# rhinempi/Reflexiv

Hardware: AMD Instinct MI355X
Metric: k-mers/sec (extract+count+filter; wall-clock to final contigs beside it) (higher is better)
Workload: dtype u64; 1 GPU; synthetic 5 Gbp in all (5 Gbp per GPU x 1), E.coli-like genome 4640000 bp (1078x), PE150, k=31, -cover 30, 0.5% substitutions; reads_per_gpu=33333334, kmer_instances_per_gpu=4000000080, distinct_kmers=352952250, kmers_kept=4639950, parallelism=1 GPU

## Files before the change

### reflexiv_amd/api.py

```python
from __future__ import annotations

import ctypes as C
from dataclasses import dataclass

import time

import numpy as np

from . import _lib
from ._lib import Params, CRecords, RfxError, TWIN_DS, TWIN_RDD, RFX_OK, RFX_E_CAP


def _p(a):
    return a.ctypes.data_as(C.c_void_p) if a is not None else None


def _cap_error(where, need, detail) -> RfxError:
    e = RfxError(RFX_E_CAP, where, detail)
    e.need = int(need)
    return e


@dataclass
class Records:
# ... 1426 lines not shown
    def comm_destroy(self):
        if getattr(self, "comm", None):
            self.L.rfx_comm_destroy(self.comm)
            self.comm = None

    def comm_all_reduce(self, vals, op: str = "sum"):
        a = (C.c_int64 * len(vals))(*[int(v) for v in vals])
        self._check(self.L.rfx_comm_all_reduce_i64(self.comm, a, len(vals), 0 if op == "sum" else 1), "rfx_comm_all_reduce_i64")
        return [int(x) for x in a]

    def sharded_count_dev(self, d_words: int, n_reads: int, words_per_read: int, read_len: int, k: int, d_out_keys: int,
                          d_out_counts: int, cap: int, min_cov=2, max_cov=10_000_000, twin=TWIN_DS, generations=4,
                          front_clip=0, end_clip=0, d_read_len: int = 0):
        n = C.c_int64(0)
        tot = (C.c_int64 * 3)()
        st = self.L.rfx_dev_sharded_count(self.ctx, self.comm, C.c_void_p(d_words), C.c_void_p(d_read_len), C.c_int64(n_reads), words_per_read,
                                          read_len, k, front_clip, end_clip, generations, min_cov, max_cov, twin,
                                          C.c_void_p(d_out_keys), C.c_void_p(d_out_counts), C.c_int64(cap), C.byref(n), tot)
        if st == RFX_E_CAP:
            e = RfxError(st, "rfx_dev_sharded_count", f"needs room for {n.value} survivors, cap is {cap}")
            e.need = int(n.value)
            raise e
        self._check(st, "rfx_dev_sharded_count")
        return int(n.value), [int(x) for x in tot]

    def sharded_assemble_dev(self, d_keys: int, d_counts: int, n: int, prm: Params, gather_below: int = -1, text_cap: int = None):
        trace = np.zeros(prm.max_iter + 8, np.int64)
        cap = (1 << 20) + 64 * max(n, 1) if text_cap is None else int(text_cap)
        self.text_retries = 0
        while True:
            buf = np.empty(max(cap, 1), np.uint8)
            ln, nc, ntr = C.c_int64(0), C.c_int64(0), C.c_int64(0)
            st = self.L.rfx_dev_sharded_assemble(self.ctx, self.comm, C.c_void_p(d_keys), C.c_void_p(d_counts), C.c_int64(n), C.byref(prm),
                                                 C.c_int64(gather_below), _p(buf), C.c_int64(cap), C.byref(ln), C.byref(nc), _p(trace),
                                                 C.c_int64(len(trace)), C.byref(ntr))
            if st == RFX_E_CAP and ln.value > cap:
                cap = int(ln.value)
                self.text_retries += 1
                continue
            self._check(st, "rfx_dev_sharded_assemble")
            return bytes(buf[:ln.value]).decode(), int(nc.value), [int(x) for x in trace[:ntr.value]]

    def sharded_assemble_reads(self, bases, read_off, prm: Params, generations: int = 4, text_cap: int = None, gather_below: int = -1):
        bases = np.ascontiguousarray(bases, np.uint8)
        read_off = np.ascontiguousarray(read_off, np.int64)
        n_reads = len(read_off) - 1
        trace = np.zeros(prm.max_iter + 8, np.int64)
        tot = (C.c_int64 * 3)()
        cap = 3 * len(bases) + (1 << 20) if text_cap is None else int(text_cap)
        self.text_retries = 0
        while True:
            buf = np.empty(max(cap, 1), np.uint8)
            ln, nc, ntr = C.c_int64(0), C.c_int64(0), C.c_int64(0)
            st = self.L.rfx_sharded_assemble_reads(self.ctx, self.comm, _p(bases), _p(read_off), C.c_int64(n_reads), C.byref(prm),
                                                   generations, C.c_int64(gather_below), _p(buf), C.c_int64(cap), C.byref(ln), C.byref(nc), _p(trace),
                                                   C.c_int64(len(trace)), C.byref(ntr), tot)
            if st == RFX_E_CAP and ln.value > cap:
                cap = int(ln.value)
                self.text_retries += 1
                continue
            self._check(st, "rfx_sharded_assemble_reads")
            return (bytes(buf[:ln.value]).decode(), int(nc.value), [int(x) for x in trace[:ntr.value]], [int(x) for x in tot])

    def comm_bytes_bucketed(self) -> int:
        return int(self.L.rfx_comm_last_bytes_bucketed(self.comm))

    def gather_shards_dev(self, d_keys: int, d_counts: int, n: int, key_words: int, count_bytes: int, root: int,
                          d_out_keys: int, d_out_counts: int, cap: int) -> int:
        m = C.c_int64(0)
        st = self.L.rfx_dev_gather_shards(self.ctx, self.comm, C.c_void_p(d_keys), C.c_void_p(d_counts), C.c_int64(n), key_words,
                                          count_bytes, root, C.c_void_p(d_out_keys), C.c_void_p(d_out_counts), C.c_int64(cap),
                                          C.byref(m))
        if st == RFX_E_CAP:
            e = RfxError(st, "rfx_dev_gather_shards", f"needs room for {m.value} entries, cap is {cap}")
            e.need = int(m.value)
            raise e
        self._check(st, "rfx_dev_gather_shards")
        return int(m.value)

    def count_timing(self):
        out = {}
        for name in ("hist1", "part1", "hist2", "part2", "hist3", "part3", "leaf", "sort", "extract_w", "count_w",
                     "pair_hist", "pair_part", "stat_leaves", "stat_passes", "stat_overflows", "stat_l2_spilled", "stat_l2_void", "stat_l2_sweeps",
                     "stat_records"):
            ms, ln = C.c_float(0), C.c_int64(0)
            if self.L.rfx_last_count_timing(self.ctx, name.encode(), C.byref(ms), C.byref(ln)) == RFX_OK:
                out[name] = (float(ms.value), int(ln.value))
        return out
```

### reflexiv_amd/csrc/rfx_kmer.hip

```cpp
#include "rfx_internal.h"
#include "rfx_device.h"
#include <algorithm>
#include <cmath>
#include <cstdlib>

using namespace rfxd;

namespace {


__device__ __forceinline__ uint64_t nuc_code(uint8_t c) {
    return c == 'A' ? 0 : c == 'C' ? 1 : c == 'G' ? 2 : 3;
}

__global__ void k_encode(const uint8_t *__restrict__ bases, const int64_t *__restrict__ read_off,
                         int64_t n_reads, int wpr, uint64_t *__restrict__ words,
                         uint32_t *__restrict__ read_len) {
    int64_t t = (int64_t)blockIdx.x * blockDim.x + threadIdx.x;
    if (t >= n_reads * wpr) return;
    int64_t r = t / wpr;
    int w = (int)(t % wpr);
    int64_t b0 = read_off[r];
    int64_t len = read_off[r + 1] - b0;
    if (w == 0 && read_len) read_len[r] = (uint32_t)len;
// ... 356 lines not shown
constexpr int LT = 768;
constexpr int LEAF_WAVES_PER_EU = 6;
constexpr int RSLOTS = 768;
constexpr int RPROBE = 4;
constexpr int LOBUF = 512;
constexpr int LOBUF1 = 128;
constexpr int WSTAGE = 160;
constexpr int LSTAGE = WSTAGE * (LT / 64);
constexpr int LCAP_BITS = 12;
constexpr int LCAP = 1 << LCAP_BITS;
__device__ __forceinline__ uint32_t leaf_slot(uint32_t g) { return g >> (32 - LCAP_BITS); }
__device__ __forceinline__ uint32_t leaf_step(uint32_t g) { return ((g >> 8) & (LCAP - 1)) | 1u; }
__device__ __forceinline__ uint32_t leaf_next(uint32_t slot, uint32_t step) { return (slot + step) & (LCAP - 1); }
constexpr int LPROBE = 48;
constexpr uint64_t EMPTY = ~0ULL;
constexpr int LSTACK = 48;
constexpr int LB = 8;
constexpr int PBLOCK = 8192;
constexpr unsigned long long NOBLK = ~0ULL;

struct CountOut {
    unsigned long long n_out;
    unsigned long long n_distinct;
    unsigned long long n_failed;
    unsigned long long n_passes;
    unsigned long long n_overflow;
    unsigned long long n_leaves;
};

struct alignas(16) Rec { uint64_t w0, w1; };
__device__ __forceinline__ int rec_len(const Rec &r) { return (int)((r.w1 >> 32) & 15) + 1; }
struct alignas(32) WRec { uint64_t b0, b1, b2, hd; };
__device__ __forceinline__ int rec_len(const WRec &r) { return (int)((r.hd >> 32) & 15) + 1; }
__device__ __forceinline__ uint32_t rec_hdr(const Rec &r) { return (uint32_t)r.w1; }

template <int ELEM> struct LeafElem;
template <> struct LeafElem<0> {
    using T = uint64_t;
    static constexpr int PER_LANE = LB;
    __device__ static __forceinline__ T none() { return 0; }
    __device__ static __forceinline__ uint64_t key(const T &e) { return e; }
    __device__ static __forceinline__ uint32_t weight(const T &) { return 1u; }
    template <class F> __device__ static __forceinline__ void for_each_kmer(const T &e, int, F &&f) { f(e); }
};
template <> struct LeafElem<2> {
    using T = Rec;
    static constexpr int PER_LANE = LB / 2;
    __device__ static __forceinline__ T none() { return Rec{0, 0}; }
    __device__ static __forceinline__ uint64_t key(const T &e) { return e.w0; }
    __device__ static __forceinline__ uint32_t weight(const T &e) { return (uint32_t)e.w1; }
};
template <> struct LeafElem<1> {
    using T = Rec;
    static constexpr int PER_LANE = 1;
    __device__ static __forceinline__ T none() { return Rec{0, 0}; }
    __device__ static __forceinline__ uint64_t key(const T &e) { return e.w0; }
    __device__ static __forceinline__ uint32_t weight(const T &) { return 1u; }
    template <class F> __device__ static __forceinline__ void for_each_kmer(const T &e, int k, F &&f) {
        const int n = rec_len(e);
        const int k2 = 2 * k;
        uint64_t fwd = e.w0 >> (64 - k2);
        uint64_t rc = revcomp(fwd, k);
        uint64_t rest = (e.w0 << k2) | (e.w1 >> (64 - k2));
        const uint64_t mask = low_mask(k);
        const int top = k2 - 2;
        for (int i = 0; i < n; i++) {
            f(fwd < rc ? fwd : rc);
            const uint64_t b = rest >> 62;
            rest <<= 2;
            fwd = ((fwd << 2) | b) & mask;
            rc = (rc >> 2) | ((b ^ 3) << top);
        }
    }
};

__device__ __forceinline__ uint32_t wave_incl_scan(uint32_t x) {
    x += (uint32_t)__builtin_amdgcn_update_dpp(0, (int)x, 0x111, 0xf, 0xf, false);
    x += (uint32_t)__builtin_amdgcn_update_dpp(0, (int)x, 0x112, 0xf, 0xf, false);
    x += (uint32_t)__builtin_amdgcn_update_dpp(0, (int)x, 0x114, 0xf, 0xf, false);
    x += (uint32_t)__builtin_amdgcn_update_dpp(0, (int)x, 0x118, 0xf, 0xf, false);
    x += (uint32_t)__builtin_amdgcn_update_dpp(0, (int)x, 0x142, 0xa, 0xf, false);
    x += (uint32_t)__builtin_amdgcn_update_dpp(0, (int)x, 0x143, 0xc, 0xf, false);
    return x;
}

template <int ELEM, int KC = 0>
__global__ __launch_bounds__(LT, LEAF_WAVES_PER_EU) void k_leaf_count(const typename LeafElem<ELEM>::T *__restrict__ keys,
                                                   const uint64_t *__restrict__ leaf_off, const uint64_t *__restrict__ leaf_end, int64_t nleaf,
                                                   const uint64_t *__restrict__ sl_begin, const uint64_t *__restrict__ sl_end,
                                                   uint64_t heavy, uint64_t n_elems, int k_rt,
                                                   int min_cov, int max_cov, int apply_filter,
                                                   uint64_t *__restrict__ out_keys, int32_t *__restrict__ out_counts,
                                                   unsigned long long cap, CountOut *__restrict__ co,
                                                   int pair_out, uint32_t presplit) {
    constexpr bool RECS = ELEM == 1;
    const int k = KC ? KC : k_rt;
    __shared__ __attribute__((aligned(16))) unsigned long long tkey[LCAP];
    __shared__ __attribute__((aligned(16))) uint32_t tcnt[LCAP];
    constexpr int OB1 = RECS ? LOBUF1 : LOBUF;
    constexpr int OB2 = RECS ? (LSTAGE * 8) / 12 : 0;
    constexpr int OBT = OB1 + OB2;
    __shared__ unsigned long long obk[OB1];
    __shared__ int32_t obc[OB1];
    __shared__ uint32_t stackS[LSTACK], stacks[LSTACK];
    __shared__ int sp;
    __shared__ uint32_t overflow, ob_n, ob_lim;
    __shared__ unsigned long long g_emit;
    __shared__ unsigned long long blk_base, blk_next;
    __shared__ uint32_t blk_pos, have_next, need_grab;
    __shared__ uint32_t ps_eff;
    __shared__ __attribute__((aligned(16))) uint64_t stage[RECS ? LSTAGE : 2];
    unsigned long long *const obk2 = (unsigned long long *)stage;
    int32_t *const obc2 = (int32_t *)(obk2 + OB2);
    auto ob_put = [&](uint32_t i, unsigned long long key, int32_t c) __attribute__((always_inline)) {
        if (OB2 == 0 || i < (uint32_t)OB1) { obk[i] = key; obc[i] = c; }
        else { obk2[i - OB1] = key; obc2[i - OB1] = c; }
    };
    static_assert(RSLOTS == 64 * (LT / 64), "one block of record slots per wave");
    __shared__ unsigned long long rA[RECS ? RSLOTS : 1], rBC[RECS ? RSLOTS : 1];
    __shared__ uint32_t agg_on, agg_saved, agg_total;
    uint32_t my_distinct = 0;
    unsigned long long my_passes = 0, my_overflows = 0;
    const int lane_ = threadIdx.x & 63;
    const int wave_ = threadIdx.x >> 6;
    constexpr int NW = LT / 64;

    const int64_t l0 = (int64_t)(((unsigned long long)blockIdx.x * (unsigned long long)nleaf) / gridDim.x);
    const int64_t l1 = (int64_t)(((unsigned long long)(blockIdx.x + 1) * (unsigned long long)nleaf) / gridDim.x);
    if (l0 >= l1) return;
    const uint64_t stream_end = n_elems;
    auto range = [&](int64_t l, uint64_t &b, uint64_t &e) __attribute__((always_inline)) {
        if (sl_begin) { b = sl_begin[l]; e = sl_end[l]; return; }
        b = leaf_off[l]; e = leaf_end[l];
        if (heavy && e - b > heavy) e = b;
    };

    for (int i = threadIdx.x; i < LCAP; i += LT) { tkey[i] = EMPTY; tcnt[i] = 0; }
    if constexpr (RECS) for (int i = threadIdx.x; i < RSLOTS; i += LT) { rA[i] = EMPTY; rBC[i] = EMPTY; }
    if (threadIdx.x == 0) {
        ob_n = 0; ob_lim = 0xffffffffu; overflow = 0; sp = 0;
        blk_base = NOBLK; blk_next = NOBLK; blk_pos = PBLOCK; have_next = 0; need_grab = 1;
        ps_eff = presplit ? presplit : 0xffffffffu;
        agg_on = 1; agg_saved = 0; agg_total = 0;
    }

    auto flush = [&]() {
        __syncthreads();
        const uint32_t cntv = ob_n < ob_lim ? ob_n : ob_lim;
        if (ob_n == 0) return;
        if (threadIdx.x == 0 && cntv) g_emit = atomicAdd(&co->n_out, (unsigned long long)cntv);
        __syncthreads();
        for (uint32_t i = threadIdx.x; i < cntv; i += LT) {
            const unsigned long long pos = g_emit + i;
            if (pos < cap) {
                const bool own = OB2 == 0 || i < (uint32_t)OB1;
                const unsigned long long key = own ? obk[i] : obk2[i - OB1];
                const int32_t c = own ? obc[i] : obc2[i - OB1];
                if (pair_out) ((Rec *)out_keys)[pos] = Rec{key, (uint64_t)(uint32_t)c};
                else { out_keys[pos] = key; out_counts[pos] = c; }
            }
        }
        __syncthreads();
        if (threadIdx.x == 0) { ob_n = 0; ob_lim = 0xffffffffu; }
        __syncthreads();
    };

// ... 1113 lines not shown
constexpr int OS_CSTRIDE = 16;
constexpr int OS_MAXG = 512;
constexpr int OS_HOLES = 3;
struct OneSweep {
    const uint64_t *reg_start;
    const uint32_t *reg_cap;
    unsigned long long *cursor;
    uint64_t *holes;
    int *overflow;
    uint64_t total;
    unsigned long long *tile_counter;
    uint32_t ose, ose_shift;
};

template <int W, int SEG = 16, bool WIDE = false>
__global__ __launch_bounds__(SKT) void k_sk_sample_hist(ReadSrc s, Level lv, int sample, unsigned long long *__restrict__ hist) {
    __shared__ uint32_t h[1 << MAX_BITS];
    const int nb = 1 << lv.bits;
    for (int i = threadIdx.x; i < nb; i += SKT) h[i] = 0;
    __syncthreads();
    const int64_t ntile = (s.n_threads + SKT - 1) / SKT;
    for (int64_t T = (int64_t)blockIdx.x * sample; T < ntile; T += (int64_t)gridDim.x * sample) {
        const int64_t g = T * SKT + threadIdx.x;
        const bool in = g < s.n_threads;
        SegPos q{0, 0};
        int nk_r = 0;
        uint64_t w[3] = {0, 0, 0}, hi, lo;
        if (in) {
            q.r = g / s.segs;
            q.sgm = (int)(g - q.r * s.segs);
            seg_load<SEG>(s, q, w);
            nk_r = read_nk<WIDE>(s, q.r);
        }
        if (SEG == 32 || in)
            seg_runs<W, SEG == 32, SEG>(s, nk_r, q.sgm, w, [&](int, int, uint32_t canon) { atomicAdd(&h[sk_digit(canon, lv)], 1u); }, &hi, &lo);
    }
    __syncthreads();
    for (int i = threadIdx.x; i < nb; i += SKT) if (h[i]) atomicAdd(&hist[i], (unsigned long long)h[i]);
}

__global__ __launch_bounds__(1024) void k_plan_regions(const unsigned long long *__restrict__ hist, int nb, double scale, int G, int cap_pct,
                                                       double tiles,
                                                       uint64_t *__restrict__ reg_start, uint32_t *__restrict__ reg_cap,
                                                       unsigned long long *__restrict__ cursor, unsigned long long *__restrict__ totals) {
    __shared__ uint64_t caps[1 << MAX_BITS];
    __shared__ unsigned long long busiest;
    __shared__ uint32_t ose_s;
    const int d = threadIdx.x;
    if (d == 0) busiest = 0;
    __syncthreads();
    if (d < nb) atomicMax(&busiest, hist[d]);
    __syncthreads();
    if (d == 0) {
        const double per_tile = (double)busiest * scale / tiles;
        ose_s = per_tile <= 16.0 ? 64u : per_tile <= 32.0 ? 128u : per_tile <= 64.0 ? 256u : 0u;
    }
    __syncthreads();
    const uint32_t E = ose_s ? ose_s : OSE_MIN;
    if (d < nb) {
        const double c = (double)hist[d];
        const double est = c * scale;
        double room = (est + 6.0 * scale * sqrt(c + 1.0) + est / 64.0 + 1024.0) * (double)cap_pct / 100.0;
        uint64_t cap = (uint64_t)room + (uint64_t)G * OS_HOLES * E;
        cap = (cap + E - 1) / E * E;
        if (cap > 0xFFFFFF00ULL) cap = 0xFFFFFF00ULL / E * E;
        caps[d] = cap;
        reg_cap[d] = (uint32_t)cap;
    }
    __syncthreads();
    if (threadIdx.x == 0) {
        uint64_t at = 0;
        for (int i = 0; i < nb; i++) { reg_start[i] = at; cursor[(size_t)i * OS_CSTRIDE] = at; at += caps[i]; }
        reg_start[nb] = at;
        totals[0] = at + E;
        totals[1] = 0;
        totals[2] = ose_s;
    }
}

template <int SEG, bool WIDE> struct OsGeo {
    static constexpr int T = SEG > 16 && !WIDE ? 512 : SKT;
};
template <int W, bool WIDE = false, int SEG = 16>
__global__ __launch_bounds__((OsGeo<SEG, WIDE>::T), WIDE || SEG > 16 ? 4 : 8) void k_sk_onesweep(ReadSrc s, Level lv, OneSweep os,
                                                               std::conditional_t<WIDE, WRec, Rec> *__restrict__ out) {
    using RT = std::conditional_t<WIDE, WRec, Rec>;
    constexpr int SKT = OsGeo<SEG, WIDE>::T;
    extern __shared__ __attribute__((aligned(32))) unsigned char sk_smem[];
    const int nb = 1 << lv.bits;
#define buf ((RT *)sk_smem)
#define tail ((uint32_t *)(sk_smem + (size_t)nb * SKB * sizeof(RT)))
#define head (tail + nb)
#define cstart (tail + 2 * nb)
#define cbase (tail + 3 * nb)
#define nbase (tail + 4 * nb)
#define pbase (tail + 5 * nb)
    constexpr uint32_t DUMP = 0xFFFFFFFFu;
    const uint32_t OSE = os.ose, OSH = os.ose_shift;
    const uint64_t dump_at = os.total - OSE;
    auto grab = [&](int d) __attribute__((always_inline)) -> uint32_t {
        const unsigned long long b = atomicAdd(&os.cursor[(size_t)d * OS_CSTRIDE], (unsigned long long)OSE);
        return b + OSE <= dump_at ? (uint32_t)(b >> OSH) : DUMP;
    };
    auto phys = [&](uint32_t v, uint32_t cs, uint32_t cb, uint32_t nx) __attribute__((always_inline)) -> uint64_t {
        const uint32_t o = v - cs;
        const uint32_t b = o < (uint32_t)OSE ? cb : nx;
        return (b == DUMP ? dump_at : (uint64_t)b << OSH) + (o & (OSE - 1));
    };
    constexpr uint32_t NONE = 0xFFFFFFFEu;
    for (int i = threadIdx.x; i < nb; i += SKT) {
        tail[i] = 0; head[i] = 0; cstart[i] = 0;
        cbase[i] = grab(i);
        nbase[i] = grab(i);
        pbase[i] = grab(i);
    }
    __syncthreads();
    constexpr int LPB = SEG > 16 || WIDE ? 4 : SKB;
    auto drain = [&](bool final) __attribute__((always_inline)) {
#pragma nounroll
        for (int d = threadIdx.x / LPB; d < nb; d += SKT / LPB) {
            const int j = threadIdx.x % LPB;
            const uint32_t h = head[d], t = tail[d], cs = cstart[d], cb = cbase[d], nx = nbase[d];
            uint32_t e, nh;
            if (t - h > (uint32_t)SKB) { e = h + SKB; nh = t; }
            else {
                e = final ? t : (t & ~(uint32_t)(SKA - 1));
                if (e < h) e = h;
                nh = e;
            }
#pragma unroll
            for (int q = 0; q < SKB / LPB; q++) {
                const uint32_t g = h + j + q * LPB;
                if (g < e) out[phys(g, cs, cb, nx)] = buf[(size_t)d * SKB + (g & (SKB - 1))];
            }
            if (j == 0) {
                head[d] = nh;
                if (nh - cs >= (uint32_t)OSE) {
                    uint32_t c = cs, b0 = cb, b1 = nx, b2 = pbase[d];
                    while (nh - c >= (uint32_t)OSE) { c += OSE; b0 = b1; b1 = b2 != NONE ? b2 : grab(d); b2 = NONE; }
                    cstart[d] = c; cbase[d] = b0; nbase[d] = b1; pbase[d] = b2;
                }
            }
        }
    };
    __shared__ long long tile_lds[2];
    const int64_t ntile = (s.n_threads + SKT - 1) / SKT;
    const int my_d = (int)threadIdx.x;
    int64_t T = blockIdx.x;
    for (int rnd = 0; T < ntile; rnd++) {
        long long t_next = 0;
        if (threadIdx.x == SKT - 1) t_next = (long long)gridDim.x + (long long)atomicAdd(os.tile_counter, 1ULL);
        const bool ask = my_d < nb && pbase[my_d] == NONE;
        uint32_t req = DUMP;
        if (ask) req = grab(my_d);
        const int64_t g = T * SKT + threadIdx.x;
        const bool in = g < s.n_threads;
        SegPos q{0, 0};
        int nk_r = 0;
        uint64_t w[3] = {0, 0, 0}, hi = 0, lo = 0;
        uint32_t past = 0;
        if (in) {
            q.r = g / s.segs;
            q.sgm = (int)(g - q.r * s.segs);
            seg_load<SEG>(s, q, w);
            nk_r = read_nk<WIDE>(s, q.r);
        }
        if (SEG == 32 || in) {
            seg_runs<W, true, SEG>(s, nk_r, q.sgm, w, [&](int i0, int n, uint32_t canon) {
                const uint64_t hh = mmer_hash64(canon);
                const uint32_t hdr = (uint32_t)((hh << OWNER_BITS) >> 32);
                const unsigned d = lv.n_owners > 0 ? (((unsigned)__umul64hi(hh, (uint64_t)lv.n_owners) << lv.sub_bits) | (hdr >> (32 - lv.sub_bits)))
                                                   : rec_digit(hdr, 0, lv.bits);
                RT r;
                if constexpr (WIDE) {
                    const uint64_t *gw = s.words + q.r * s.wpr;
                    const int p = s.fc - s.wfl + q.sgm * SEG + i0;
                    const int wi = p >> 5, sft = 2 * (p & 31), last = s.wpr - 1;
                    const uint64_t a0 = gw[wi < last ? wi : last], a1 = gw[wi + 1 < last ? wi + 1 : last];
                    const uint64_t a2 = gw[wi + 2 < last ? wi + 2 : last], a3 = gw[wi + 3 < last ? wi + 3 : last];
                    r.b0 = sft ? (a0 << sft) | (a1 >> (64 - sft)) : a0;
                    r.b1 = sft ? (a1 << sft) | (a2 >> (64 - sft)) : a1;
                    r.b2 = sft ? (a2 << sft) | (a3 >> (64 - sft)) : a2;
                    r.hd = ((uint64_t)(n - 1) << 32) | (uint64_t)hdr;
                } else {
                    const int sft = 2 * i0;
                    const uint64_t x = (uint64_t)past << 32;
                    r.w0 = sft ? (hi << sft) | (lo >> (64 - sft)) : hi;
                    r.w1 = ((sft ? (lo << sft) | (x >> (64 - sft)) : lo) & 0xFFFFFFF000000000ULL) | ((uint64_t)(n - 1) << 32) | (uint64_t)hdr;
                }
                const uint32_t pos = atomicAdd(&tail[d], 1u);
                if (pos - head[d] < (uint32_t)SKB) buf[(size_t)d * SKB + (pos & (SKB - 1))] = r;
                else {
                    const uint32_t cs = cstart[d];
                    if (pos - cs < 2u * OSE) out[phys(pos, cs, cbase[d], nbase[d])] = r;
                    else *os.overflow = 1;
                }
            }, &hi, &lo, nullptr, &past);
        }
        if (threadIdx.x == SKT - 1) tile_lds[rnd & 1] = t_next;
        if (ask) pbase[my_d] = req;
        __syncthreads();
        drain(false);
        T = tile_lds[rnd & 1];
        __syncthreads();
    }
    drain(true);
    __syncthreads();
    for (int d = threadIdx.x; d < nb; d += SKT) {
        const uint32_t used = tail[d] - cstart[d], cb = cbase[d], nx = nbase[d], px = pbase[d];
        uint64_t *hl = os.holes + ((size_t)d * gridDim.x + blockIdx.x) * OS_HOLES;
        hl[0] = cb != DUMP && used < OSE ? ((((uint64_t)cb << OSH) + used) << 16) | (uint64_t)(OSE - used) : 0;
        hl[1] = nx != DUMP ? (((uint64_t)nx << OSH) << 16) | (uint64_t)OSE : 0;
        hl[2] = px != DUMP && px != NONE ? (((uint64_t)px << OSH) << 16) | (uint64_t)OSE : 0;
    }
}
#undef buf
#undef tail
#undef head
#undef cstart
#undef cbase
#undef nbase
#undef pbase

constexpr int FH_T = 1024;
template <class RT>
__global__ __launch_bounds__(FH_T) void k_fix_holes(OneSweep os, int G, RT *__restrict__ out, uint64_t *__restrict__ seg_begin,
                                                   uint64_t *__restrict__ seg_end, unsigned long long *__restrict__ totals) {
    constexpr int NHMAX = 2048;
    static_assert(NHMAX >= OS_HOLES * OS_MAXG && NHMAX % FH_T == 0, "holes per bucket");
    constexpr int NWMAX = NHMAX * OSE_MAX / 32;
    __shared__ uint32_t hstart[NHMAX], hoff[NHMAX + 1];
    __shared__ uint32_t bitmap[NWMAX];
    __shared__ uint32_t wsum[FH_T / 64];
    const int d = blockIdx.x;
    const int NH = OS_HOLES * G;
    const uint64_t base = os.reg_start[d];
    const unsigned long long alloc = os.cursor[(size_t)d * OS_CSTRIDE] - base;
    if (alloc > (unsigned long long)os.reg_cap[d]) {
        if (threadIdx.x == 0) { seg_begin[d] = base; seg_end[d] = base; *os.overflow = 1; }
        return;
    }
    auto block_excl_scan = [&](uint32_t v, uint32_t *total) __attribute__((always_inline)) -> uint32_t {
        const int lane = threadIdx.x & 63, wave = threadIdx.x >> 6;
        uint32_t x = v;
#pragma unroll
        for (int o = 1; o < 64; o <<= 1) { const uint32_t y = __shfl_up(x, o, 64); if (lane >= o) x += y; }
        if (lane == 63) wsum[wave] = x;
        __syncthreads();
        uint32_t b = 0, tot = 0;
        for (int i = 0; i < FH_T / 64; i++) { const uint32_t sv = wsum[i]; if (i < wave) b += sv; tot += sv; }
        __syncthreads();
        *total = tot;
        return b + x - v;
    };
    constexpr int HPT = NHMAX / FH_T;
    uint32_t hs[HPT], hl[HPT];
    uint32_t mine = 0;
#pragma unroll
    for (int r = 0; r < HPT; r++) {
        const int t = threadIdx.x * HPT + r;
        const uint64_t x = t < NH ? os.holes[(size_t)d * NH + t] : 0;
        hl[r] = (uint32_t)(x & 0xFFFFu);
        hs[r] = hl[r] ? (uint32_t)((x >> 16) - base) : 0u;
        mine += hl[r];
    }
    uint32_t H;
    block_excl_scan(mine, &H);
    const uint32_t size = (uint32_t)alloc - H;
    const uint32_t nw = (H + 31) / 32;
    const uint32_t wpt = (nw + FH_T - 1) / FH_T;
    for (uint32_t i = threadIdx.x; i < nw; i += FH_T) bitmap[i] = 0;
    __syncthreads();
    uint32_t fill[HPT], fsum = 0;
#pragma unroll
    for (int r = 0; r < HPT; r++) {
        fill[r] = hs[r] < size ? (hs[r] + hl[r] <= size ? hl[r] : size - hs[r]) : 0u;
        fsum += fill[r];
        for (uint32_t p = hs[r] + fill[r]; p < hs[r] + hl[r]; p++) atomicOr(&bitmap[(p - size) >> 5], 1u << ((p - size) & 31));
    }
    uint32_t F;
    uint32_t fo = block_excl_scan(fsum, &F);
#pragma unroll
    for (int r = 0; r < HPT; r++) {
        const int t = threadIdx.x * HPT + r;
        hstart[t] = hs[r]; hoff[t] = fo; fo += fill[r];
    }
// ... 255 lines not shown
            else return level_digit<MODE>(Rec{a.x, a.y}, used, lv);
        };
#define RCL_COUNT(i) { const uint64_t idx = c0 + (uint64_t)(i) * WCT + threadIdx.x; d##i = digit_of(q##i, w##i); if (idx < qe) atomicAdd(&h[d##i], 1u); }
        RCL_COUNT(0) RCL_COUNT(1) RCL_COUNT(2) RCL_COUNT(3)
#undef RCL_COUNT
        __syncthreads();
        for (int d = threadIdx.x; d < nb; d += WCT) {
            const uint32_t c = h[d];
            const uint64_t rs = pl.reg_start[d], re = pl.reg_start[d + 1];
            unsigned long long base = 0;
            if (c) base = atomicAdd(&pl.cursor[d], (unsigned long long)c);
            tail[d] = head[d] = rs + base;
            lim[d] = re;
        }
        __syncthreads();
#define RCL_PUT(i) { const uint64_t idx = c0 + (uint64_t)(i) * WCT + threadIdx.x; \
            if (idx < qe) { \
                const unsigned d = d##i; \
                const unsigned long long g = atomicAdd(&tail[d], 1ULL); \
                if (g >= lim[d]) {  } \
                else if (g - head[d] < (unsigned long long)B) { V *to = (V *)buf + ((size_t)d * B + (g & (B - 1))) * NV; to[0] = q##i; if constexpr (NV == 2) to[1] = w##i; } \
                else { V *to = (V *)out + g * NV; to[0] = q##i; if constexpr (NV == 2) to[1] = w##i; } \
            } }
        RCL_PUT(0) RCL_PUT(1) RCL_PUT(2) RCL_PUT(3)
#undef RCL_PUT
        __syncthreads();
        drain(true);
        __syncthreads();
    }
}

constexpr int L2S_STRIDE = 16;
struct L2Plan {
    const uint64_t *seg_begin, *seg_end; const uint64_t *child_start; int *flags;
    void *spill_rec; uint32_t *spill_child; unsigned long long *spill_cursor; uint32_t spill_cap;
    unsigned long long *tail_cursor; uint64_t out_cap;
};
template <int MODE>
__global__ __launch_bounds__(PT) void k_l2_sample(const typename LevelElem<MODE>::T *__restrict__ recs, L2Plan pl, Level lv, int used,
                                                  uint32_t *__restrict__ sampled) {
    __shared__ uint32_t h[1 << MAX_BITS];
    const int p = blockIdx.x, nb = 1 << lv.bits;
    for (int i = threadIdx.x; i < nb; i += PT) h[i] = 0;
    __syncthreads();
    const uint64_t qb = pl.seg_begin[p], qe = pl.seg_end[p];
    for (uint64_t c = (uint64_t)blockIdx.y * L2S_STRIDE; c * PT < qe - qb; c += (uint64_t)gridDim.y * L2S_STRIDE) {
        const uint64_t i = qb + c * PT + threadIdx.x;
        if (i < qe) {
            const typename LevelElem<MODE>::T r = recs[i];
            if constexpr (MODE == 2) { if (r.w1 == 0) continue; }
            atomicAdd(&h[level_digit<MODE>(r, used, lv)], 1u);
        }
    }
    __syncthreads();
    for (int i = threadIdx.x; i < nb; i += PT) if (h[i]) atomicAdd(&sampled[(int64_t)p * nb + i], h[i]);
}
__global__ void k_l2_caps(const uint32_t *__restrict__ sampled, int64_t nchild, uint32_t *__restrict__ ccap, int pct) {
    const int64_t c = (int64_t)blockIdx.x * blockDim.x + threadIdx.x;
    if (c >= nchild) return;
    const float s = (float)sampled[c];
    uint32_t C = (uint32_t)((float)L2S_STRIDE * (s + 6.0f * sqrtf(s + 1.0f) + 32.0f));
    if (pct != 100) C = (uint32_t)((uint64_t)C * (uint64_t)pct / 100u);
    ccap[c] = (C + 7u) & ~7u;
}
__global__ __launch_bounds__(1024) void k_l2_check(L2Plan pl, int nseg, int64_t nchild, uint64_t out_cap) {
    __shared__ unsigned long long sum_n, mx_n;
    if (threadIdx.x == 0) { sum_n = 0; mx_n = 0; }
    __syncthreads();
    if ((int)threadIdx.x < nseg) {
        const unsigned long long n = pl.seg_end[threadIdx.x] - pl.seg_begin[threadIdx.x];
        atomicAdd(&sum_n, n);
        atomicMax(&mx_n, n);
    }
    __syncthreads();
    if (threadIdx.x == 0) {
        const unsigned long long mean = sum_n / (unsigned long long)(nseg > 0 ? nseg : 1);
        pl.flags[0] = (pl.child_start[nchild] + 8ULL * pl.spill_cap + 65536ULL > out_cap || mx_n > mean + mean / 2 + 4096) ? 1 : 0;
        pl.flags[1] = 0;
        *pl.spill_cursor = 0;
        *pl.tail_cursor = (pl.child_start[nchild] + 7ULL) & ~7ULL;
    }
}

typedef unsigned long long l2_v2 __attribute__((ext_vector_type(2)));
template <class RT>
__device__ __forceinline__ RT l2_load_stream(const RT *p) {
    static_assert(sizeof(RT) == 16 || sizeof(RT) == 32, "16- or 32-byte records");
    const l2_v2 a = __builtin_nontemporal_load((const l2_v2 *)p);
    if constexpr (sizeof(RT) == 32) {
        const l2_v2 b = __builtin_nontemporal_load((const l2_v2 *)p + 1);
        return RT{a.x, a.y, b.x, b.y};
    } else return RT{a.x, a.y};
}
template <class RT>
__device__ __forceinline__ void l2_store_stream(RT *p, const RT &r) {
    const uint64_t *w = (const uint64_t *)&r;
    __builtin_nontemporal_store(l2_v2{w[0], w[1]}, (l2_v2 *)p);
    if constexpr (sizeof(RT) == 32) __builtin_nontemporal_store(l2_v2{w[2], w[3]}, (l2_v2 *)p + 1);
}
template <int B, int MODE>
__global__ __launch_bounds__(WCT) void k_rec_l2sweep(const typename LevelElem<MODE>::T *__restrict__ recs, L2Plan pl, Level lv, int used,
                                                     typename LevelElem<MODE>::T *__restrict__ out, uint64_t *__restrict__ leaf_end) {
    using Rec = typename LevelElem<MODE>::T;
    extern __shared__ __attribute__((aligned(32))) unsigned char wc_smem[];
    constexpr int A = B / 2;
    if (pl.flags[0]) return;
    const int p = blockIdx.x;
    const int nb = 1 << lv.bits;
    const uint64_t qb = pl.seg_begin[p], qe = pl.seg_end[p];
    Rec *buf = (Rec *)wc_smem;
    unsigned long long *tail = (unsigned long long *)(buf + (size_t)nb * B);
    unsigned long long *head = tail + nb;
    unsigned long long *lim = head + nb;
    for (int i = threadIdx.x; i < nb; i += WCT) {
        tail[i] = head[i] = pl.child_start[(int64_t)p * nb + i];
        lim[i] = pl.child_start[(int64_t)p * nb + i + 1];
    }
    __syncthreads();
    auto drain = [&](bool final) __attribute__((always_inline)) {
#pragma nounroll
        for (int d = threadIdx.x / B; d < nb; d += WCT / B) {
            const int j = threadIdx.x % B;
            const unsigned long long h = head[d], lm = lim[d];
            unsigned long long t = tail[d];
            if (t > lm) t = lm;
            unsigned long long e, nh;
            if (t - h > (unsigned long long)B) { e = h + B; nh = t; }
            else {
                e = final ? t : (t & ~(unsigned long long)(A - 1));
                if (e < h) e = h;
                nh = e;
            }
            const unsigned long long g = h + j;
            if (g < e) l2_store_stream(out + g, buf[(size_t)d * B + (g & (B - 1))]);
            if (j == 0) head[d] = nh;
        }
    };
    for (uint64_t b0 = qb; b0 < qe; b0 += (uint64_t)WCT * WC_PER) {
        Rec r[WC_PER];
#pragma unroll
        for (int i = 0; i < WC_PER; i++) {
            const uint64_t idx = b0 + (uint64_t)i * WCT + threadIdx.x;
            r[i] = l2_load_stream(recs + (idx < qe ? idx : qe - 1));
        }
#pragma unroll
        for (int i = 0; i < WC_PER; i++) {
            const uint64_t idx = b0 + (uint64_t)i * WCT + threadIdx.x;
            bool live = idx < qe;
            if constexpr (MODE == 2) live = live && r[i].w1 != 0;
            if (live) {
                const unsigned d = level_digit<MODE>(r[i], used, lv);
                const unsigned long long g = atomicAdd(&tail[d], 1ULL);
                if (g >= lim[d]) {
                    const unsigned long long sk = atomicAdd(pl.spill_cursor, 1ULL);
                    if (sk < (unsigned long long)pl.spill_cap) { ((Rec *)pl.spill_rec)[sk] = r[i]; pl.spill_child[sk] = (uint32_t)(p * nb + (int)d); }
                    else pl.flags[1] = 1;
                }
                else if (g - head[d] < (unsigned long long)B) buf[(size_t)d * B + (g & (B - 1))] = r[i];
                else out[g] = r[i];
            }
        }
        __syncthreads();
        drain(false);
        __syncthreads();
    }
    drain(true);
    __syncthreads();
    for (int d = threadIdx.x; d < nb; d += WCT) leaf_end[(int64_t)p * nb + d] = tail[d];
}

constexpr int L2F_T = 1024, L2F_SLOTS = 2048, L2F_MAXC = 1536;
template <class RT>
__global__ __launch_bounds__(L2F_T) void k_l2_spill_fix(L2Plan pl, uint64_t *__restrict__ cstart, uint64_t *__restrict__ lend, RT *__restrict__ out) {
    __shared__ uint32_t tkey[L2F_SLOTS], tcnt[L2F_SLOTS], tfill[L2F_SLOTS], tcap[L2F_SLOTS];
    __shared__ unsigned long long tbase[L2F_SLOTS];
    __shared__ uint32_t ndistinct;
    __shared__ int bad;
    if (pl.flags[0] || pl.flags[1]) return;
    const unsigned long long ns = *pl.spill_cursor;
    if (ns == 0) return;
    constexpr uint32_t NOKEY = 0xFFFFFFFFu;
    for (int i = threadIdx.x; i < L2F_SLOTS; i += L2F_T) { tkey[i] = NOKEY; tcnt[i] = 0; tfill[i] = 0; }
// ... 743 lines not shown
    const int OST = seg32 ? OsGeo<32, false>::T : SKT;
    const int64_t ntile = ceil_div(rsrc.n_threads, OST);
    const int64_t ntile_s = ceil_div(rsrc.n_threads, SKT);
    const int per_cu = WIDE ? 1 : 2;
    const int G = (int)std::max<int64_t>(1, std::min<int64_t>(std::min<int64_t>(OS_MAXG, (int64_t)ctx->num_cu * per_cu),
                                                                std::max<int64_t>(std::min<int64_t>(ntile, 64), ntile / 32)));
    int sample = 32;
    if (ntile_s < 64 * (int64_t)sample) sample = (int)std::max<int64_t>(1, ntile_s / 64);
    const int64_t n_sampled = ceil_div(ntile_s, sample);
    const int cap_pct = getenv("RFX_SK_ONESWEEP_CAP") ? std::max(1, atoi(getenv("RFX_SK_ONESWEEP_CAP"))) : 100;
    DevBuf hist, reg_start, reg_cap, cursor, totals, holes;
    RFX_HIP(hist.alloc((size_t)nb * 8 + 16, ctx->stream));
    RFX_ALLOC(reg_start, uint64_t, nb + 1);
    RFX_ALLOC(reg_cap, uint32_t, nb);
    RFX_ALLOC(cursor, unsigned long long, (size_t)nb * OS_CSTRIDE);
    RFX_HIP(totals.alloc(24, ctx->stream));
    RFX_ALLOC(holes, uint64_t, (size_t)nb * OS_HOLES * G);
    RFX_HIP(hipMemsetAsync(hist.p, 0, (size_t)nb * 8 + 16, ctx->stream));
    int *d_overflow = (int *)(hist.as<unsigned long long>() + nb);
    {
        ScopedTimer t(ctx, hn);
        const dim3 gs((unsigned)std::min<int64_t>(n_sampled, (int64_t)ctx->num_cu * 8));
        if constexpr (WIDE) {
            if (W == 18) RFX_LAUNCH((k_sk_sample_hist<18, 16, true>), gs, dim3(SKT), 0, rsrc, lv, sample, hist.as<unsigned long long>());
            else RFX_LAUNCH((k_sk_sample_hist<19, 16, true>), gs, dim3(SKT), 0, rsrc, lv, sample, hist.as<unsigned long long>());
        } else switch (W) {
#define X(w) case w: if (seg32) RFX_LAUNCH((k_sk_sample_hist<w, 32>), gs, dim3(SKT), 0, rsrc, lv, sample, hist.as<unsigned long long>()); \
                     else RFX_LAUNCH((k_sk_sample_hist<w>), gs, dim3(SKT), 0, rsrc, lv, sample, hist.as<unsigned long long>()); break;
            RFX_SK_W_CASES(X)
            default: X(19)
#undef X
        }
        RFX_LAUNCH(k_plan_regions, dim3(1), dim3(1024), 0, hist.as<unsigned long long>(), nb,
                   (double)ntile_s / (double)n_sampled, G, cap_pct, (double)ntile, reg_start.as<uint64_t>(), reg_cap.as<uint32_t>(),
                   cursor.as<unsigned long long>(), totals.as<unsigned long long>());
    }
    unsigned long long h_tot[3] = {0, 0, 0};
    RFX_HIP(hipMemcpyAsync(h_tot, totals.p, 24, hipMemcpyDeviceToHost, ctx->stream));
    RFX_TRY(sync_checked(ctx));
    const uint32_t ose = (uint32_t)h_tot[2];
    if (ose == 0) {
        if (getenv("RFX_TRACE")) fprintf(stderr, "one-sweep level 1: not tried (the sample puts too much on one bucket)\n");
        return RFX_OK;
    }
    int ose_shift = 0;
    while ((1u << ose_shift) < ose) ose_shift++;
    Rec *dst = d_dst;
    if (d_dst) {
        if ((int64_t)h_tot[0] > cap_dst) { *n_recs = (int64_t)h_tot[0]; return RFX_E_CAP; }
    } else {
        dst = (Rec *)ctx->ws_get(ws_slot, (size_t)h_tot[0] * sizeof(Rec));
        if (!dst) { ctx->last_error = "workspace allocation failed"; return RFX_E_HIP; }
    }
    const OneSweep os{reg_start.as<uint64_t>(), reg_cap.as<uint32_t>(), cursor.as<unsigned long long>(), holes.as<uint64_t>(), d_overflow,
                      (uint64_t)h_tot[0], hist.as<unsigned long long>() + nb + 1, ose, (uint32_t)ose_shift};
    const size_t lds = (size_t)nb * (SKB * sizeof(Rec) + 24);
    {
        ScopedTimer t(ctx, pn);
        if constexpr (WIDE) {
            if (W == 18) {
                RFX_HIP(hipFuncSetAttribute((const void *)k_sk_onesweep<18, true>, hipFuncAttributeMaxDynamicSharedMemorySize, (int)lds));
                RFX_LAUNCH((k_sk_onesweep<18, true>), dim3((unsigned)G), dim3(SKT), lds, rsrc, lv, os, dst);
            } else {
                RFX_HIP(hipFuncSetAttribute((const void *)k_sk_onesweep<19, true>, hipFuncAttributeMaxDynamicSharedMemorySize, (int)lds));
                RFX_LAUNCH((k_sk_onesweep<19, true>), dim3((unsigned)G), dim3(SKT), lds, rsrc, lv, os, dst);
            }
        } else {
            switch (W) {
#define X(w) case w: if (seg32) { \
                         RFX_HIP(hipFuncSetAttribute((const void *)k_sk_onesweep<w, false, 32>, hipFuncAttributeMaxDynamicSharedMemorySize, (int)lds)); \
                         RFX_LAUNCH((k_sk_onesweep<w, false, 32>), dim3((unsigned)G), dim3(OST), lds, rsrc, lv, os, dst); \
                     } else { \
                         RFX_HIP(hipFuncSetAttribute((const void *)k_sk_onesweep<w>, hipFuncAttributeMaxDynamicSharedMemorySize, (int)lds)); \
                         RFX_LAUNCH((k_sk_onesweep<w>), dim3((unsigned)G), dim3(SKT), lds, rsrc, lv, os, dst); \
                     } break;
                RFX_SK_W_CASES(X)
                default: X(19)
#undef X
            }
        }
        RFX_LAUNCH(k_fix_holes<Rec>, dim3((unsigned)nb), dim3(FH_T), 0, os, G, dst, d_seg_begin, d_seg_end,
                   totals.as<unsigned long long>());
    }
    int h_over = 0;
    RFX_HIP(hipMemcpyAsync(h_tot, totals.p, 16, hipMemcpyDeviceToHost, ctx->stream));
    RFX_HIP(hipMemcpyAsync(&h_over, d_overflow, 4, hipMemcpyDeviceToHost, ctx->stream));
    RFX_TRY(sync_checked(ctx));
    if (getenv("RFX_TRACE"))
        fprintf(stderr, "one-sweep level 1: %llu records in regions of %llu (sample 1/%d, %d workgroups, extents of %u)%s\n", h_tot[1], h_tot[0], sample, G, ose,
                h_over ? " -- a region overflowed: two passes instead" : "");
    if (h_over == 2) { ctx->last_error = "one-sweep level 1: holes and tail records do not balance"; return RFX_E_STATE; }
    if (h_over) return RFX_OK;
    *out_recs = dst;
    *n_recs = (int64_t)h_tot[1];
    ctx->timing["stat_records"].launches += (int64_t)h_tot[1];
    *done = true;
    return RFX_OK;
}

template <int MODE>
static int records_resweep(rfx_ctx *ctx, const typename LevelElem<MODE>::T *recs, int64_t n_recs, const Level &lv, int used, int oslot,
                           uint64_t *d_seg_begin, uint64_t *d_seg_end, const typename LevelElem<MODE>::T **out_recs, bool *done,
                           const char *hn, const char *pn) {
    using RT = typename LevelElem<MODE>::T;
    *done = false;
    const int mode = getenv("RFX_REC_ONESWEEP") ? atoi(getenv("RFX_REC_ONESWEEP")) : (MODE == 0 || MODE == 3 ? 1 : 0);
    if (MODE == 2 || !mode || lv.bits < 4 || lv.bits > 9 || lv.n_owners > 0 || (mode != 2 && n_recs < ((int64_t)1 << 24))) return RFX_OK;
    const int nb = 1 << lv.bits;
    constexpr int B = MODE == 3 ? 8 : 16;
    if (nb > 256 && B * sizeof(RT) * nb + 28 * (size_t)nb > 160 * 1024) return RFX_OK;
    const size_t lds = (size_t)nb * (B * sizeof(RT) + 28);
    const int64_t nchunk = ceil_div(n_recs, PT);
    int sample = 32;
    if (nchunk < 256 * (int64_t)sample) sample = (int)std::max<int64_t>(1, nchunk / 256);
    const int64_t n_sampled = ceil_div(nchunk, sample);
    DevBuf hist, reg_start, cursor;
    RFX_HIP(hist.alloc((size_t)nb * 8 + 8, ctx->stream));
    RFX_ALLOC(reg_start, uint64_t, nb + 1);
    RFX_ALLOC(cursor, unsigned long long, nb);
    RFX_HIP(hipMemsetAsync(hist.p, 0, (size_t)nb * 8 + 8, ctx->stream));
    const ClaimPlan pl{reg_start.as<uint64_t>(), cursor.as<unsigned long long>(), (int *)(hist.as<unsigned long long>() + nb)};
    {
        ScopedTimer t(ctx, hn);
        RFX_LAUNCH(k_rec_sample_hist<MODE>, dim3((unsigned)std::min<int64_t>(n_sampled, (int64_t)ctx->num_cu * 8)), dim3(PT), 0,
                   recs, (uint64_t)n_recs, lv, used, sample, hist.as<unsigned long long>());
        RFX_LAUNCH(k_claim_plan, dim3(1), dim3(1024), 0, hist.as<unsigned long long>(), nb,
                   (double)nchunk / (double)n_sampled, pl);
    }
    uint64_t total = 0;
    RFX_HIP(hipMemcpyAsync(&total, reg_start.as<uint64_t>() + nb, 8, hipMemcpyDeviceToHost, ctx->stream));
    RFX_TRY(sync_checked(ctx));
    if ((int64_t)total > 2 * n_recs + ((int64_t)1 << 26)) return RFX_OK;
    RT *dst = (RT *)ctx->ws_get(oslot, (size_t)total * sizeof(RT));
    if (!dst) { ctx->last_error = "workspace allocation failed"; return RFX_E_HIP; }
    {
        ScopedTimer t(ctx, pn);
        constexpr int64_t CHUNK = (int64_t)RCL_TILES * WCT * WC_PER;
        RFX_HIP(hipFuncSetAttribute((const void *)k_rec_claim_scatter<B, MODE>, hipFuncAttributeMaxDynamicSharedMemorySize, (int)lds));
        const int per_cu = lds <= 72 * 1024 ? 2 : 1;
        RFX_LAUNCH((k_rec_claim_scatter<B, MODE>), dim3((unsigned)std::min<int64_t>(ceil_div(n_recs, CHUNK), (int64_t)ctx->num_cu * per_cu)), dim3(WCT), lds, recs, (uint64_t)n_recs, lv, used,
                   pl, dst);
        RFX_LAUNCH(k_claim_ends, dim3((unsigned)ceil_div(nb, 256)), dim3(256), 0, pl, nb, d_seg_begin, d_seg_end);
    }
    int h_over = 0;
    RFX_HIP(hipMemcpyAsync(&h_over, pl.overflow, 4, hipMemcpyDeviceToHost, ctx->stream));
    RFX_TRY(sync_checked(ctx));
    if (getenv("RFX_TRACE"))
        fprintf(stderr, "record level without a histogram: %lld records in regions of %llu (sample 1/%d)%s\n", (long long)n_recs, (unsigned long long)total,
                sample, h_over ? " -- a bucket outgrew its region: the exact form instead" : "");
    if (h_over) return RFX_OK;
    *out_recs = dst;
    *done = true;
    return RFX_OK;
}

template <int MODE>
static int partition_record_levels(rfx_ctx *ctx, const typename LevelElem<MODE>::T *recs, int64_t n_recs, int ws_slot_of_recs,
                                   const std::vector<int> &bits, size_t first_level, int used, DevBuf **seg_cur_io,
                                   DevBuf **seg_next_io, int64_t *nseg_io, const typename LevelElem<MODE>::T **cur_out,
                                   const uint64_t *seg_end_first = nullptr, DevBuf *seg_end_buf = nullptr,
                                   const uint64_t **seg_end_out = nullptr) {
    using Rec = typename LevelElem<MODE>::T;
    DevBuf *seg_cur = *seg_cur_io, *seg_next = *seg_next_io;
    int64_t nseg = *nseg_io;
    const Rec *cur = recs;
    int slot = ws_slot_of_recs;
    const uint64_t *seg_end_cur = seg_end_first;
    if (seg_end_out) *seg_end_out = nullptr;
    for (size_t l = first_level; l < bits.size(); l++) {
        Level lv{};
// ... 986 lines not shown
```

Baseline: 205.1 billion k-mers/s.

## Prefetch next tile and overlap atomics in one-sweep kernel, stream stores

```diff
diff --git a/reflexiv_amd/api.py b/reflexiv_amd/api.py
--- a/reflexiv_amd/api.py
+++ b/reflexiv_amd/api.py
@@ -1532,7 +1532,7 @@
         out = {}
         for name in ("hist1", "part1", "hist2", "part2", "hist3", "part3", "leaf", "sort", "extract_w", "count_w",
                      "pair_hist", "pair_part", "stat_leaves", "stat_passes", "stat_overflows", "stat_l2_spilled", "stat_l2_void", "stat_l2_sweeps",
-                     "stat_records"):
+                     "stat_records", "stat_l1_void_rounds"):
             ms, ln = C.c_float(0), C.c_int64(0)
             if self.L.rfx_last_count_timing(self.ctx, name.encode(), C.byref(ms), C.byref(ln)) == RFX_OK:
                 out[name] = (float(ms.value), int(ln.value))
diff --git a/reflexiv_amd/csrc/rfx_kmer.hip b/reflexiv_amd/csrc/rfx_kmer.hip
--- a/reflexiv_amd/csrc/rfx_kmer.hip
+++ b/reflexiv_amd/csrc/rfx_kmer.hip
@@ -462,6 +462,23 @@
     x += (uint32_t)__builtin_amdgcn_update_dpp(0, (int)x, 0x142, 0xa, 0xf, false);
     x += (uint32_t)__builtin_amdgcn_update_dpp(0, (int)x, 0x143, 0xc, 0xf, false);
     return x;
+}
+
+typedef unsigned long long l2_v2 __attribute__((ext_vector_type(2)));
+template <class RT>
+__device__ __forceinline__ RT l2_load_stream(const RT *p) {
+    static_assert(sizeof(RT) == 16 || sizeof(RT) == 32, "16- or 32-byte records");
+    const l2_v2 a = __builtin_nontemporal_load((const l2_v2 *)p);
+    if constexpr (sizeof(RT) == 32) {
+        const l2_v2 b = __builtin_nontemporal_load((const l2_v2 *)p + 1);
+        return RT{a.x, a.y, b.x, b.y};
+    } else return RT{a.x, a.y};
+}
+template <class RT>
+__device__ __forceinline__ void l2_store_stream(RT *p, const RT &r) {
+    const uint64_t *w = (const uint64_t *)&r;
+    __builtin_nontemporal_store(l2_v2{w[0], w[1]}, (l2_v2 *)p);
+    if constexpr (sizeof(RT) == 32) __builtin_nontemporal_store(l2_v2{w[2], w[3]}, (l2_v2 *)p + 1);
 }
 
 template <int ELEM, int KC = 0>
@@ -1741,7 +1758,7 @@
     static constexpr int T = SEG > 16 && !WIDE ? 512 : SKT;
 };
 template <int W, bool WIDE = false, int SEG = 16>
-__global__ __launch_bounds__((OsGeo<SEG, WIDE>::T), WIDE || SEG > 16 ? 4 : 8) void k_sk_onesweep(ReadSrc s, Level lv, OneSweep os,
+__global__ __launch_bounds__((OsGeo<SEG, WIDE>::T), 4) void k_sk_onesweep(ReadSrc s, Level lv, OneSweep os,
                                                                std::conditional_t<WIDE, WRec, Rec> *__restrict__ out) {
     using RT = std::conditional_t<WIDE, WRec, Rec>;
     constexpr int SKT = OsGeo<SEG, WIDE>::T;
@@ -1757,9 +1774,11 @@
     constexpr uint32_t DUMP = 0xFFFFFFFFu;
     const uint32_t OSE = os.ose, OSH = os.ose_shift;
     const uint64_t dump_at = os.total - OSE;
+    auto extent_of = [&](unsigned long long b) __attribute__((always_inline)) -> uint32_t {
+        return b + OSE <= dump_at ? (uint32_t)(b >> OSH) : DUMP;
+    };
     auto grab = [&](int d) __attribute__((always_inline)) -> uint32_t {
-        const unsigned long long b = atomicAdd(&os.cursor[(size_t)d * OS_CSTRIDE], (unsigned long long)OSE);
-        return b + OSE <= dump_at ? (uint32_t)(b >> OSH) : DUMP;
+        return extent_of(atomicAdd(&os.cursor[(size_t)d * OS_CSTRIDE], (unsigned long long)OSE));
     };
     auto phys = [&](uint32_t v, uint32_t cs, uint32_t cb, uint32_t nx) __attribute__((always_inline)) -> uint64_t {
         const uint32_t o = v - cs;
@@ -1790,14 +1809,13 @@
 #pragma unroll
             for (int q = 0; q < SKB / LPB; q++) {
                 const uint32_t g = h + j + q * LPB;
-                if (g < e) out[phys(g, cs, cb, nx)] = buf[(size_t)d * SKB + (g & (SKB - 1))];
+                if (g < e) l2_store_stream(out + phys(g, cs, cb, nx), buf[(size_t)d * SKB + (g & (SKB - 1))]);
             }
             if (j == 0) {
                 head[d] = nh;
                 if (nh - cs >= (uint32_t)OSE) {
-                    uint32_t c = cs, b0 = cb, b1 = nx, b2 = pbase[d];
-                    while (nh - c >= (uint32_t)OSE) { c += OSE; b0 = b1; b1 = b2 != NONE ? b2 : grab(d); b2 = NONE; }
-                    cstart[d] = c; cbase[d] = b0; nbase[d] = b1; pbase[d] = b2;
+                    const uint32_t b2 = pbase[d];
+                    cstart[d] = cs + OSE; cbase[d] = nx; nbase[d] = final && b2 == NONE ? DUMP : b2; pbase[d] = NONE;
                 }
             }
         }
@@ -1806,24 +1824,31 @@
     const int64_t ntile = (s.n_threads + SKT - 1) / SKT;
     const int my_d = (int)threadIdx.x;
     int64_t T = blockIdx.x;
+    auto fetch = [&](int64_t tile, SegPos &q, int &nk_r, uint64_t (&w)[3]) __attribute__((always_inline)) {
+        const int64_t g = tile * SKT + threadIdx.x;
+        const int64_t gc = g < s.n_threads ? g : s.n_threads - 1;
+        q.r = gc / s.segs;
+        q.sgm = (int)(gc - q.r * s.segs);
+        seg_load<SEG>(s, q, w);
+        nk_r = read_nk<WIDE>(s, q.r);
+    };
+    int64_t T1 = (int64_t)gridDim.x + blockIdx.x;
+    SegPos qn{0, 0};
+    int nkn = 0;
+    uint64_t wn[3] = {0, 0, 0};
+    if (T < ntile) fetch(T, qn, nkn, wn);
+    asm volatile("" : "+v"(wn[0]), "+v"(wn[1]), "+v"(wn[2]), "+v"(nkn));
     for (int rnd = 0; T < ntile; rnd++) {
-        long long t_next = 0;
-        if (threadIdx.x == SKT - 1) t_next = (long long)gridDim.x + (long long)atomicAdd(os.tile_counter, 1ULL);
+        const bool in = T * SKT + threadIdx.x < s.n_threads;
+        SegPos q{in ? qn.r : 0, in ? qn.sgm : 0};
+        int nk_r = in ? nkn : 0;
+        uint64_t w[3] = {in ? wn[0] : 0, in ? wn[1] : 0, in ? wn[2] : 0}, hi = 0, lo = 0;
+        uint32_t past = 0;
+        unsigned long long t_raw = 0, req_raw = 0;
         const bool ask = my_d < nb && pbase[my_d] == NONE;
-        uint32_t req = DUMP;
-        if (ask) req = grab(my_d);
-        const int64_t g = T * SKT + threadIdx.x;
-        const bool in = g < s.n_threads;
-        SegPos q{0, 0};
-        int nk_r = 0;
-        uint64_t w[3] = {0, 0, 0}, hi = 0, lo = 0;
-        uint32_t past = 0;
-        if (in) {
-            q.r = g / s.segs;
-            q.sgm = (int)(g - q.r * s.segs);
-            seg_load<SEG>(s, q, w);
-            nk_r = read_nk<WIDE>(s, q.r);
-        }
+        if (ask) req_raw = atomicAdd(&os.cursor[(size_t)my_d * OS_CSTRIDE], (unsigned long long)OSE);
+        fetch(T1, qn, nkn, wn);
+        if (threadIdx.x == SKT - 1) t_raw = atomicAdd(os.tile_counter, 1ULL);
         if (SEG == 32 || in) {
             seg_runs<W, true, SEG>(s, nk_r, q.sgm, w, [&](int i0, int n, uint32_t canon) {
                 const uint64_t hh = mmer_hash64(canon);
@@ -1842,25 +1867,33 @@
                     r.b2 = sft ? (a2 << sft) | (a3 >> (64 - sft)) : a2;
                     r.hd = ((uint64_t)(n - 1) << 32) | (uint64_t)hdr;
                 } else {
-                    const int sft = 2 * i0;
-                    const uint64_t x = (uint64_t)past << 32;
-                    r.w0 = sft ? (hi << sft) | (lo >> (64 - sft)) : hi;
-                    r.w1 = ((sft ? (lo << sft) | (x >> (64 - sft)) : lo) & 0xFFFFFFF000000000ULL) | ((uint64_t)(n - 1) << 32) | (uint64_t)hdr;
+                    const uint32_t d0 = (uint32_t)(hi >> 32), d1 = (uint32_t)hi, d2 = (uint32_t)(lo >> 32), d3 = (uint32_t)lo;
+                    const uint32_t e0 = d0 >> 1, e1 = __builtin_amdgcn_alignbit(d0, d1, 1), e2 = __builtin_amdgcn_alignbit(d1, d2, 1);
+                    const uint32_t e3 = __builtin_amdgcn_alignbit(d2, d3, 1), e4 = __builtin_amdgcn_alignbit(d3, past, 1);
+                    const bool up = i0 >= 16;
+                    const uint32_t a0 = up ? e1 : e0, a1 = up ? e2 : e1, a2 = up ? e3 : e2, a3 = up ? e4 : e3;
+                    const uint32_t sh = 31u - 2u * ((uint32_t)i0 & 15u);
+                    const uint32_t w0h = __builtin_amdgcn_alignbit(a0, a1, sh), w0l = __builtin_amdgcn_alignbit(a1, a2, sh);
+                    const uint32_t w1h = (__builtin_amdgcn_alignbit(a2, a3, sh) & 0xFFFFFFF0u) | (uint32_t)(n - 1);
+                    r.w0 = ((uint64_t)w0h << 32) | w0l;
+                    r.w1 = ((uint64_t)w1h << 32) | (uint64_t)hdr;
                 }
                 const uint32_t pos = atomicAdd(&tail[d], 1u);
                 if (pos - head[d] < (uint32_t)SKB) buf[(size_t)d * SKB + (pos & (SKB - 1))] = r;
                 else {
                     const uint32_t cs = cstart[d];
                     if (pos - cs < 2u * OSE) out[phys(pos, cs, cbase[d], nbase[d])] = r;
-                    else *os.overflow = 1;
+                    else { os.overflow[0] = 1; os.overflow[1] = 1; }
                 }
             }, &hi, &lo, nullptr, &past);
         }
-        if (threadIdx.x == SKT - 1) tile_lds[rnd & 1] = t_next;
-        if (ask) pbase[my_d] = req;
+        asm volatile("" : "+v"(wn[0]), "+v"(wn[1]), "+v"(wn[2]), "+v"(nkn), "+v"(t_raw), "+v"(req_raw));
+        if (threadIdx.x == SKT - 1) tile_lds[rnd & 1] = 2LL * (long long)gridDim.x + (long long)t_raw;
+        if (ask) pbase[my_d] = extent_of(req_raw);
         __syncthreads();
         drain(false);
-        T = tile_lds[rnd & 1];
+        T = T1;
+        T1 = tile_lds[rnd & 1];
         __syncthreads();
     }
     drain(true);
@@ -2282,22 +2315,6 @@
     }
 }
 
-typedef unsigned long long l2_v2 __attribute__((ext_vector_type(2)));
-template <class RT>
-__device__ __forceinline__ RT l2_load_stream(const RT *p) {
-    static_assert(sizeof(RT) == 16 || sizeof(RT) == 32, "16- or 32-byte records");
-    const l2_v2 a = __builtin_nontemporal_load((const l2_v2 *)p);
-    if constexpr (sizeof(RT) == 32) {
-        const l2_v2 b = __builtin_nontemporal_load((const l2_v2 *)p + 1);
-        return RT{a.x, a.y, b.x, b.y};
-    } else return RT{a.x, a.y};
-}
-template <class RT>
-__device__ __forceinline__ void l2_store_stream(RT *p, const RT &r) {
-    const uint64_t *w = (const uint64_t *)&r;
-    __builtin_nontemporal_store(l2_v2{w[0], w[1]}, (l2_v2 *)p);
-    if constexpr (sizeof(RT) == 32) __builtin_nontemporal_store(l2_v2{w[2], w[3]}, (l2_v2 *)p + 1);
-}
 template <int B, int MODE>
 __global__ __launch_bounds__(WCT) void k_rec_l2sweep(const typename LevelElem<MODE>::T *__restrict__ recs, L2Plan pl, Level lv, int used,
                                                      typename LevelElem<MODE>::T *__restrict__ out, uint64_t *__restrict__ leaf_end) {
@@ -3207,10 +3224,12 @@
         RFX_LAUNCH(k_fix_holes<Rec>, dim3((unsigned)nb), dim3(FH_T), 0, os, G, dst, d_seg_begin, d_seg_end,
                    totals.as<unsigned long long>());
     }
-    int h_over = 0;
+    int h_flag[2] = {0, 0};
     RFX_HIP(hipMemcpyAsync(h_tot, totals.p, 16, hipMemcpyDeviceToHost, ctx->stream));
-    RFX_HIP(hipMemcpyAsync(&h_over, d_overflow, 4, hipMemcpyDeviceToHost, ctx->stream));
+    RFX_HIP(hipMemcpyAsync(h_flag, d_overflow, 8, hipMemcpyDeviceToHost, ctx->stream));
     RFX_TRY(sync_checked(ctx));
+    const int h_over = h_flag[0];
+    if (h_flag[1]) ctx->timing["stat_l1_void_rounds"].launches += 1;
     if (getenv("RFX_TRACE"))
         fprintf(stderr, "one-sweep level 1: %llu records in regions of %llu (sample 1/%d, %d workgroups, extents of %u)%s\n", h_tot[1], h_tot[0], sample, G, ose,
                 h_over ? " -- a region overflowed: two passes instead" : "");
```

Measured after the change: 212.9 billion k-mers/s (median of 6 runs). +3.8%, better.
